# gabraham/flashpca

Measured on AMD Instinct MI355X. Metric: genotype cells/sec (N x P x iters) for k=20 PCA, higher is better.
Workload: dtype i8 (integer genotypes x 7 byte slices of the f64 operand; exact i32 accumulation, f64 recombination; agrees with the f64 kernels to ~3e-15, see fp64_mode); 1 GPU; cfg3: synthetic 500000 samples x 100000 SNPs total, SNP-sharded across GPUs, k=20 (BASELINE configs[2]/[3]); samples=500000, snps_total=100000, snps_per_gpu=100000, k=20, blockvec=16, solver_default_blockvec=16, parallelism=snp-shard x1 + all-reduce(N x b) [single]

## Files before the change

### flashpca_amd/_lib.py

```python
import ctypes as C
import os
import subprocess

HERE = os.path.dirname(os.path.abspath(__file__))
LIB_PATH = os.environ.get("FPCA_LIB") or os.path.join(HERE, "_build", "libfpca.so")
if LIB_PATH == "testhooks":
    LIB_PATH = os.path.join(HERE, "_build", "testhooks", "libfpca.so")
CLI_PATH = os.path.join(HERE, "_build", "flashpca")
HOOKS_LIB_PATH = os.path.join(HERE, "_build", "testhooks", "libfpca.so")
HOOKS_CLI_PATH = os.path.join(HERE, "_build", "testhooks", "flashpca")
CSRC = os.path.join(HERE, "csrc")

STANDARDISE = {"binom": 2, "binom2": 3}
STANDARDISE_DENSE = {"none": 0, "sd": 1, "binom": 2, "binom2": 3, "center": 4}
DIVISOR = {"none": 0, "n1": 1, "p": 2}
UNIQUE_ID_BYTES = 128
SCCA_STATUS = {0: "ok", 1: "maxiter reached", 2: "lambda1 too large", 3: "lambda2 too large"}

ALLREDUCE_FN = C.CFUNCTYPE(C.c_int, C.c_void_p, C.c_void_p, C.c_uint64, C.c_void_p)
COLLECTIVE_FN = C.CFUNCTYPE(C.c_int, C.c_void_p, C.c_void_p, C.c_void_p, C.c_uint64, C.c_void_p)


class PcaOpts(C.Structure):
    _fields_ = [
# ... 115 lines not shown
    "fpca_set_total_snps": (_I, [_P, _U64]),
    "fpca_set_rank": (_I, [_P, _I, _I]),
    "fpca_collective_stats": (_I, [_P, C.POINTER(_U64), C.POINTER(_U64)]),
    "fpca_pca_init_opts": (None, [C.POINTER(PcaOpts), C.c_size_t, C.c_size_t]),
    "fpca_pca_row_ranges": (_I, [_P, C.POINTER(PcaOpts), C.POINTER(_U64), _I]),
    "fpca_pca": (_I, [_P, C.POINTER(PcaOpts), _P, _P, _P, _P, _P, _P, C.POINTER(PcaInfo)]),
    "fpca_check": (_I, [_P, _P, C.c_int64, _P, _I, _I, _P, C.POINTER(_D), C.POINTER(_D)]),
    "fpca_ucca": (_I, [_P, _P, C.c_int64, _I, _I, _P, C.c_int64]),
    "fpca_scca_prepare": (_I, [_P, _P, C.c_int64, _I, _I, _I]),
    "fpca_scca_fit": (_I, [_P, _D, _D, _I, _I, _D, _P, C.c_int64, _P, C.c_int64, _P, C.c_int64, _P, _P, C.c_int64, _P, C.c_int64,
                           C.POINTER(_I), _P, _P, _P, C.POINTER(_I)]),
    "fpca_scca_cv": (_I, [_P, _P, C.c_int64, _I, _P, _I, _P, _I, _P, _I, _I, _I, _I, _I, _D, _P, C.c_int64, C.c_int64, _D, _I, _P, _P, _P, _P, _P, _P,
                          C.POINTER(_D), C.POINTER(_D), C.POINTER(_D), _P, _P]),
    "fpca_bench_apply": (_I, [_P, _I, _I, _I, C.POINTER(BenchResult)]),
    "fpca_profile_begin": (_I, [_P, _I]),
    "fpca_profile_sample_every": (_I, [_P, _I]),
    "fpca_profile_end": (_I, [_P, _I, C.POINTER(BenchResult), C.POINTER(_I)]),
    "fpca_bench_stats": (_I, [_P, _I, C.POINTER(_D), C.POINTER(_D)]),
    "fpca_debug_mfma_probe": (_I, [_P, _P, _P]),
    "fpca_debug_mfma_i8_probe": (_I, [_P, _P, _P]),
    "fpca_debug_mfma_peak": (_I, [_I, _I, _I, C.POINTER(_D)]),
    "fpca_debug_k4": (_I, [_P, _I, _I, _P, _P, _P, _P, _I, _P, _P]),
    "fpca_debug_k4_bench": (_I, [_P, _I, _I, _I, C.POINTER(_D), C.POINTER(_D)]),
    "fpca_debug_k4_fused": (_I, [_P, _I, _I, _P, _P, _P, _P, _P]),
    "fpca_debug_k4_fused_bench": (_I, [_P, _I, _I, _I, C.POINTER(_D)]),
    "fpca_debug_k4_inplace": (_I, [_P, _I, _I, _P, _P, _P, _I, _P, _P]),
    "fpca_debug_fp_plan": (_I, [_P, _I, C.POINTER(_I)]),
    "fpca_debug_poison_partials": (_I, [_P]),
    "fpca_debug_missing_lists": (_I, [_P, _I, _I, _P, _P, _U64, C.POINTER(_U64)]),
    "fpca_debug_gather": (_I, [_I, _I, _P, _P, _U64, _P, _U64, _P, _P, _P, _U64, _U64, _I, _D, _P, C.POINTER(_I)]),
    "fpca_debug_i8_nsc_pad": (_I, [_I, _I, C.POINTER(_I)]),
    "fpca_debug_i8_slices": (_I, [_I, _I, _I, _U64, _U64, _U64, _P, _P, _P, _P, _I, C.POINTER(SlicesOut), C.POINTER(SlicesOut), C.POINTER(_I)]),
    "fpca_debug_i8_instances": (_I, [_P, _I, C.POINTER(_I)]),
    "fpca_debug_f_sf":(_I, [_D, _U64, _I, C.POINTER(_D), C.POINTER(_D)]),
    "fpca_debug_fold_stats": (_I, [_P, _P, _I, _P, _I, _P]),
    "fpca_debug_snp_qc_rule": (_I, [_P, _P, _U64, _U64, _D, _D, _P, C.POINTER(_U64)]),
    "fpca_debug_snp_subset_bench": (_I, [_P, _P, _I, C.POINTER(_D), C.POINTER(_D)]),
    "fpca_debug_ld_prune_rule": (_I, [_P, _U64, C.c_uint32, C.c_uint32, _P, _P, _P, _P, C.POINTER(_U64)]),
    "fpca_bench_ld": (_I, [_P, C.c_uint32, _I, _P, C.POINTER(_D)]),
    "fpca_debug_king_rule": (_I, [_P, _P, _U64, _U64, _P, C.POINTER(_U64)]),
    "fpca_bench_king": (_I, [_P, _I, _P, C.POINTER(_D)]),
    "fpca_debug_sample_qc_rule": (_I, [_P, _U64, _U64, _D, _P, C.POINTER(_U64)]),
    "fpca_debug_snp_qc_counts_rule": (_I, [_P, _P, _U64, _U64, _D, _D, _D, _P, C.POINTER(_U64)]),
    "fpca_bench_qc": (_I, [_P, _I, _P, C.POINTER(_D)]),
    "fpca_debug_scratch_live": (_I, [C.POINTER(_U64)]),
    "fpca_debug_scratch_fail_at": (_I, [_U64]),
}

ABI_VERSION = 4

_lib = None
_loaded = {}


def _load(path):
    if path not in _loaded:
        if not os.path.exists(path):
            raise RuntimeError(
                "%s not found -- build it with `make -C flashpca_amd/csrc` (or __graft_entry__.build()); this package has "
                "no CPU fallback" % path
            )
        L = C.CDLL(path)
        try:
            L.fpca_abi_version.restype = C.c_int
            abi = L.fpca_abi_version()
        except AttributeError:
# ... 49 lines not shown
```

### flashpca_amd/csrc/kernels.hpp

```cpp
#pragma once
#include <hip/hip_runtime.h>

#include <cstddef>
#include <cstdint>

namespace fpca {
namespace kern {

void repitch(const uint8_t *src, uint64_t np, uint64_t nrec, uint8_t *dst, size_t pitch, hipStream_t stream);
void fix_last_byte(uint8_t *packed, size_t pitch, uint64_t np, int valid_in_last, uint64_t P_g, hipStream_t stream);
void gather_records(const uint8_t *src, size_t pitch, const uint32_t *idx, uint64_t nrec, uint8_t *dst, hipStream_t stream);
void ld_totals(const uint8_t *packed, size_t pitch, uint64_t nrec, uint32_t *tot, hipStream_t stream);
void ld_band(const uint8_t *packed, size_t pitch, const uint32_t *tot, uint32_t npad, uint64_t i0, uint64_t ni, uint64_t jend, uint32_t span,
             double *r2, uint32_t *bits, uint32_t words, double thr, bool force_general, hipStream_t stream);

void bed_stats(const uint8_t *packed, size_t pitch, uint64_t N, uint64_t P_g, int stand_method, double *lut,
               double *mean, double *sd, double *sumsq, uint32_t *nmiss , hipStream_t stream);
void lut_from_meansd(const double *mean, const double *sd, uint64_t P_g, double *lut, hipStream_t stream);

void xt_b(const uint8_t *packed, size_t pitch, const double *lut, const double *B, double *Tpart, uint64_t N_pad,
          uint64_t P_pad, int b, int nsplit, bool fp32, hipStream_t stream);
void x_t(const uint8_t *packed, size_t pitch, const double *lut, const double *T, double *Ypart, uint64_t N_pad,
         uint64_t P_pad, int b, int nsplit, bool fp32, hipStream_t stream);
void reduce_sum(const double *part, double *out, uint64_t count, int nsplit, hipStream_t stream);
// ... 39 lines not shown
void synth_generate(uint8_t *packed, size_t pitch, uint64_t N, uint64_t snp_begin, uint64_t P_g, uint64_t seed,
                    int n_pop, uint32_t fst_fp, uint32_t miss_thr, hipStream_t stream, int maf_model = 0, int missing_model = 0,
                    uint32_t conc_fp = 0, uint64_t med_q32 = 0, uint32_t sig2_fp = 0);

void mfma_layout_probe(const double *A, const double *B, double *D, hipStream_t stream);

double mfma_peak_tflops(int waves_per_simd, int iters, int pattern, hipStream_t stream);

constexpr int I8_SHARDS = 8, I8_CS_STRIDE = 640;
struct SliceOp {
   const double *rowscale;
   unsigned long long *maxbits;
   int8_t *Q;
   double *colw;
   long long *colsum;
   double *copy64;
   float *copy32;
};
void i8_colmax(const double *V, uint64_t rows, int b, int nops, const SliceOp *ops, hipStream_t stream);
void i8_slice(const double *V, uint64_t rows_pad, uint64_t rows, int b, int S, int nops, const SliceOp *ops, hipStream_t stream);
void i8_maxbits_fold(const unsigned long long *bits, double *out64, hipStream_t stream);
void i8_maxbits_set(const double *all, int G, unsigned long long *bits, hipStream_t stream);
void i8_slice_rows(const double *V, uint64_t rows, int b, int S, const SliceOp &op, int8_t *Qrm, hipStream_t stream);
void i8_unpack_slices(const int8_t *Qrm, uint64_t rows_pad, int b, int S, const SliceOp &op, hipStream_t stream, uint64_t rows_valid = 0,
                      float *copy32 = nullptr, double *copy64 = nullptr);
void i8_dequant_rows(const int8_t *Qrm, uint64_t rows, int b, int S, const SliceOp &op, float *copy32, double *copy64, hipStream_t stream);
__host__ __device__ inline size_t packed_piece_offset(uint64_t r, uint64_t q, size_t pitch, bool tiled)
{
   if (!tiled) return (size_t)(r * pitch + q * 16);
   const uint64_t c = q >> 2, kh = (q >> 1) & 1, h = q & 1;
   return (size_t)((r >> 5) * 32 * pitch + c * 2048 + (h * 64 + kh * 32 + (r & 31)) * 16);
}
int gemm_i8_nsc_pad(int S, int b);
size_t gemm_i8_workspace_doubles(uint64_t rows_pad, uint64_t k_pad, int S, int b, bool two);
int gemm_i8_instances(int (*out)[6], int cap);
void gemm_i8(const uint8_t *packed, size_t pitch, const int8_t *Qg, const int8_t *Qm, const double *wg, const double *wm,
             const long long *colsum_m, const double *mean, const double *sd, double *out, double *ws, uint64_t rows_pad, uint64_t k_pad,
             uint64_t rows_valid, int mode ,
             const double *eplane , int b, int S,
             const SliceOp *next_ops, hipStream_t stream, hipEvent_t *gemm_events = nullptr, hipEvent_t before_combine = nullptr,
             bool e_only = false ,
             bool tiled = false );
void i8_rowscales(const double *mean, const double *sd, uint64_t P_g, uint64_t P_pad, double *inv_sd, double *mu_inv_sd,
                  hipStream_t stream);
void transpose_packed(const uint8_t *in, size_t pitch_in, uint64_t N_pad, uint64_t P_pad, uint8_t *out, size_t pitch_out,
                      hipStream_t stream, bool tiled = false );
void tile_packed(const uint8_t *in, size_t pitch, uint64_t rows, uint8_t *out, hipStream_t stream);
double mfma_i8_peak_tops(int waves_per_simd, int iters, uint32_t fill, hipStream_t stream);
void mfma_i8_probe(const int8_t *A, const int8_t *Bt, int *D, hipStream_t stream);

void gather_packed_rows(const uint8_t *src, size_t pitch, const uint32_t *idx, uint32_t nidx, uint32_t rows_out, uint8_t *dst, hipStream_t stream);
void patch_missing_rows(uint8_t *packed, size_t pitch, const uint32_t *idx, uint32_t nidx, hipStream_t stream);
void scatter_packed_rows(const uint8_t *src, size_t pitch, const uint32_t *idx, uint32_t nidx, uint8_t *packed, hipStream_t stream);
void gather_scaled_rows(const double *V, const double *scale, const uint32_t *idx, uint32_t nidx, uint64_t rows_out, int b, double *dst, hipStream_t stream);
void scatter_rows(const double *src, const uint32_t *idx, uint32_t nidx, int b, double *dst, hipStream_t stream);
void count_missing(const uint8_t *packed, size_t pitch, uint64_t ncols, uint64_t nrec, uint32_t *cnt, hipStream_t stream, bool tiled = false);
void fill_missing(const uint8_t *packed, size_t pitch, uint64_t ncols, uint64_t nrec, const uint32_t *ptr, uint32_t *idx, hipStream_t stream,
                  bool tiled = false);
void sparse_rows_sum(const uint32_t *ptr, const uint32_t *idx, const double *V, const double *rowscale, int b, uint64_t nrec,
                     uint64_t rows_out, double *out, hipStream_t stream, const double *init = nullptr ,
                     bool short_lists = false ,
                     double avg_len = 0 );
void sparse_rows_sum_f32(const uint32_t *ptr, const uint32_t *idx, const float *V, const double *colw, int b, uint64_t nrec, uint64_t rows_out,
                         double *out, hipStream_t stream, const double *init = nullptr, bool short_lists = false, double avg_len = 0);
int sparse_rows_sum_variant(int b, bool rowscale, bool short_lists, double avg_len);

}
// ... 2 lines not shown
```

### flashpca_amd/csrc/kernels_i8.hip

```cpp
#include <hip/hip_runtime.h>

#include <algorithm>
#include <cmath>
#include <cstdio>
#include <cstdlib>
#include <type_traits>
#include <utility>

#include "common.hpp"
#include "dev_scratch.hpp"
#include "kernels.hpp"
#include "launch_check.hpp"

namespace fpca {
namespace kern {

typedef int v4i __attribute__((ext_vector_type(4)));
typedef int v16i __attribute__((ext_vector_type(16)));
typedef double d2 __attribute__((ext_vector_type(2)));
typedef uint32_t u4 __attribute__((ext_vector_type(4)));
typedef uint32_t u2 __attribute__((ext_vector_type(2)));



// ... 448 lines not shown
   static constexpr int SEGS = KC / 16, RSTEP = THREADS / SEGS;
   static constexpr bool HALF8 = HALF && RSTEP == 32;
   static constexpr int NP1 = HALF8 ? (COLS - 16) / RSTEP + 1 : COLS / RSTEP;
   static constexpr int NP = NQ * NP1;
   static constexpr int KS = KC / 32;
   static constexpr int PW = KC / 128;
   static constexpr int NSTEP = KS * MT * G;
   static constexpr int H = NSTEP / 2;
   static constexpr int LDS_EPI = WAVES * NT * 4096 + 2 * WC * NT * 32 * 8;
   static constexpr int LDS_NEED = (NBUF * STAGE > LDS_EPI) ? NBUF * STAGE : LDS_EPI;
   static constexpr int LDS_BYTES = (!TWO && NT <= 2 && WAVES == 4 && LDS_NEED < 56 * 1024) ? 56 * 1024 : LDS_NEED;
   static_assert((HALF8 ? (COLS - 16) % RSTEP == 0 && KC == 256 : COLS % RSTEP == 0) && NSTEP % 2 == 0 && LDS_BYTES <= 160 * 1024, "staging");
   static_assert(!HALF || RSTEP == 16 || HALF8, "the remainder tile is the last staging piece");
};

template <int MODE>
__device__ __forceinline__ bool i8_decode(uint32_t w, v4i &ag, v4i &am, uint32_t tab1)
{
   const uint32_t tabG = MODE == I8_NO_MISSING ? tab1 : 0x00010002u, tabM = 0x00000100u;
#pragma unroll
   for (int q = 0; q < 4; q++) {
      const uint32_t sel = (w >> (2 * q)) & 0x03030303u;
      ag[q] = (int)__builtin_amdgcn_perm(0u, tabG, sel);
      if (MODE != I8_NO_MISSING) am[q] = (int)__builtin_amdgcn_perm(0u, tabM, sel);
   }
   if (MODE == I8_SKIP_EMPTY)
      return __builtin_amdgcn_ballot_w64(((w & ~(w >> 1)) & 0x55555555u) != 0u) != 0ull;
   return true;
}

template <class C>
__global__ __launch_bounds__(C::THREADS, 1) void k_gemm_i8(const uint8_t *__restrict__ packed, size_t pitch,
                                                     const int8_t *__restrict__ Qg, const int8_t *__restrict__ Qm,
                                                     uint64_t k_pad, const double *__restrict__ wg, const double *__restrict__ wm, int bw,
                                                     double *__restrict__ part, uint64_t rows_pad, int chunks_total, int zb,
                                                     int nA, int sB, int cpsB, uint64_t rowB0, uint64_t rowsB, uint32_t tab1)
{
   constexpr bool TWO = C::TWO;
   constexpr int MODE = C::MODE, MATS = C::MATS;
   constexpr int MT = C::MT, NT = C::NT, NQ = C::NQ, KC = C::KC, NP = C::NP, NP1 = C::NP1, NSTEP = C::NSTEP, LDQ = C::LDQ,
                 H = C::H, G = C::G, PW = C::PW, NPK = MT * PW, NTF = C::NTF;
   constexpr bool HALF = C::HALF;
   constexpr int NBUF = C::NBUF;
   constexpr int AMASK = HALF ? 3 : 1;
   extern __shared__ __attribute__((aligned(16))) unsigned char smem[];
   const int tid = threadIdx.x, lane = tid & 63, wave = tid >> 6;
   const int li = lane & 31, kh = lane >> 5;
   const int wr = wave / C::WC, wc = wave % C::WC;
   const int rtiles = (int)((rows_pad + (C::WAVES == 8 ? C::ROWS - 1 : 0)) / C::ROWS), rtl = (rtiles + 7) / 8, ids = 8 * rtl * zb, nB = ids - nA;
   int w0 = blockIdx.x, split = 0, c_begin = 0, c_end = chunks_total;
   if (w0 >= nA) {
      const int wp = w0 - nA;
      split = wp / nB;
      w0 = nA + wp % nB;
      c_begin = split * cpsB;
      c_end = c_begin + cpsB < chunks_total ? c_begin + cpsB : chunks_total;
   }
   const int xcd = w0 & 7, sidx = w0 >> 3;
   const int zblk = sidx % zb, rt = (sidx / zb) * 8 + xcd;
   if (rt >= rtiles || c_begin >= c_end) return;
   const uint64_t row0 = (uint64_t)rt * C::ROWS;
   const int col0 = zblk * C::COLS;
   const bool idle = C::WAVES == 8 && __builtin_amdgcn_readfirstlane((int)(row0 + (uint64_t)(wr * 32 * MT) >= rows_pad)) != 0;

   v16i acc[MATS][MT][NT];
   v4i acch[MATS][MT][2];
#pragma unroll
// ... 236 lines not shown
                     acc[1][m][n] = __builtin_amdgcn_mfma_i32_32x32x32_i8(am[akey & AMASK], bq[bkey & 1][NQ - 1][j], acc[1][m][n], 0, 0, 0);
               });
            }
         }
         __builtin_amdgcn_sched_barrier(0);
         if constexpr (bkey1 != bkey) {
            wait_b(std::integral_constant<int, g1>{}, std::integral_constant<int, (bkey1 & 1)>{});
            __builtin_amdgcn_sched_barrier(0);
         }
         if constexpr (ahead) {
            wait_b(i0, i0);
            __builtin_amdgcn_sched_barrier(0);
         }
      });
      if constexpr (NBUF == 3) {
         asm volatile("s_waitcnt lgkmcnt(0)" ::: "memory");
         __builtin_amdgcn_s_barrier();
         asm volatile("" ::: "memory");
         __builtin_amdgcn_sched_barrier(0);
         buf = bufn;
      } else {
#pragma unroll
         for (int m = 0; m < MT; m++)
#pragma unroll
            for (int h = 0; h < PW; h++) {
               vm_wait<0>(pkn[m][h]);
               pk[m][h] = pkn[m][h];
            }
         __syncthreads();
      }
   }

   const int tile0 = (col0 + wc * 32 * NT) / 32;
   double *out = (split == 0 ? part + (((size_t)zblk * rows_pad + row0 + wr * 32 * MT) * 2) * bw
                             : part + (size_t)zb * rows_pad * 2 * bw +
                                  ((((size_t)(split - 1) * zb + zblk) * rowsB + (row0 - rowB0) + wr * 32 * MT) * 2) * bw) +
                 li;
   __syncthreads();
   constexpr int WREG = NT * 4096;
   double *sW = reinterpret_cast<double *>(smem + C::WAVES * WREG);
   constexpr int WCOLS = C::WC * NT * 32;
   for (int t = tid; t < WCOLS; t += C::THREADS) {
      sW[t] = t < C::COLS ? wg[col0 + t] : 0.0;
      sW[WCOLS + t] = t < C::COLS ? wm[col0 + t] : 0.0;
   }
   __syncthreads();
   static_assert(C::LDS_BYTES >= C::WAVES * WREG + 2 * WCOLS * 8, "epilogue LDS layout");
   if (idle) return;
   int *sT = reinterpret_cast<int *>(smem + wave * WREG);
   const double *sWl = sW + wc * 32 * NT + li;
   const int kb = bw / 32;
#pragma unroll
   for (int a = 0; a < MATS; a++)
#pragma unroll
      for (int m = 0; m < MT; m++) {
#pragma unroll
         for (int n = 0; n < NTF; n++) {
            const v16i v = acc[a][m][n];
#pragma unroll
            for (int r = 0; r < 16; r++) sT[(n * 32 + (r & 3) + 8 * (r >> 2) + 4 * kh) * 32 + li] = v[r];
            __builtin_amdgcn_sched_barrier(0);
         }
         if constexpr (HALF) {
#pragma unroll
            for (int t = 0; t < 2; t++)
#pragma unroll
               for (int r = 0; r < 4; r++) {
                  const int row = 16 * t + 4 * (lane >> 4) + r;
                  sT[(NTF * 32 + row) * 32 + (lane & 15)] = acch[a][m][t][r];
                  sT[(NTF * 32 + row) * 32 + 16 + (lane & 15)] = 0;
               }
         }
         __builtin_amdgcn_fence(__ATOMIC_RELEASE, "wavefront");
         __builtin_amdgcn_wave_barrier();
         for (int j = 0; j < 16; j++) {
            const int row = 16 * kh + j;
            for (int k = 0; k < kb; k++) {
               double acc64 = 0.0;
               for (int n = NT - 1 - ((NT - 1 - k) % kb); n >= 0; n -= kb)
                  acc64 += sWl[a * WCOLS + 32 * n] * (double)sT[(n * 32 + row) * 32 + li];
               out[((size_t)(32 * m + row) * 2 + a) * bw + 32 * ((tile0 + k) % kb)] = acc64;
            }
         }
         __builtin_amdgcn_fence(__ATOMIC_ACQUIRE, "wavefront");
         __builtin_amdgcn_wave_barrier();
      }
}

__global__ __launch_bounds__(256) void k_i8_combine(const double *__restrict__ part, int zb, int rows_tile, int nA, int sB, uint64_t rowB0,
                                                     uint64_t rowsB, uint64_t rows_pad, uint64_t rows_valid, int mats,
                                                     const double *__restrict__ eplane ,
                                                     int b, int bw, int S,
                                                     const double *__restrict__ wm, const long long *__restrict__ colsum_m ,
                                                     const double *__restrict__ mean, const double *__restrict__ sd,
                                                     double *__restrict__ out, const double *__restrict__ rs0,
                                                     unsigned long long *__restrict__ bits0, const double *__restrict__ rs1,
                                                     unsigned long long *__restrict__ bits1)
{
   __shared__ double smax[256], sw[9 * 64], sones[64];
   const int c = threadIdx.x % b, r_in = threadIdx.x / b, r_step = 256 / b;
   double m0 = 0.0, m1 = 0.0;
   for (int t = threadIdx.x; t < S * b; t += 256) sw[t] = (mats < 0 || !colsum_m) ? 0.0 : wm[t] * (double)colsum_fold(colsum_m, t);
   __syncthreads();
   if ((int)threadIdx.x < b) {
      double o = 0.0;
      for (int s = S - 1; s >= 0; s--) o += sw[s * b + threadIdx.x];
      sones[threadIdx.x] = o;
   }
   __syncthreads();
   if (r_in < r_step) {
      const double ones = sones[c];
      for (uint64_t row = (uint64_t)blockIdx.x * r_step + r_in; row < rows_pad; row += (uint64_t)gridDim.x * r_step) {
         double accg = 0.0, acce = 0.0;
         const int rt = (int)(row / rows_tile);
         for (int z = 0; z < zb; z++) {
            const int w0 = ((rt >> 3) * zb + z) * 8 + (rt & 7);
            const int np = w0 < nA ? 1 : sB;
            for (int p = 0; p < np; p++) {
               const double *q = p == 0 ? part + (((size_t)z * rows_pad + row) * 2) * bw
                                        : part + (size_t)zb * rows_pad * 2 * bw + ((((size_t)(p - 1) * zb + z) * rowsB + (row - rowB0)) * 2) * bw;
               for (int j = c; j < bw; j += b) {
                  accg += q[j];
                  if (mats == 2) acce += q[bw + j];
               }
            }
         }
         if (mats == 1) acce = row >= rows_valid ? ones : (eplane ? eplane[row * b + c] : 0.0);
         const double accm = ones - acce;
         double v;
         if (mats < 0)
            v = row < rows_valid ? accg : 0.0;
         else if (mean) {
            const double sdv = sd[row];
            v = (sdv > 1e-9) ? (accg - mean[row] * accm) / sdv : 0.0;
         } else
            v = accg - accm;
         out[row * b + c] = v;
         if (bits0) {
            m0 = fmax(m0, fabs(v * rs0[row]));
            m1 = fmax(m1, fabs(v * rs1[row]));
         }
      }
   }
   if (bits0) {
      colmax_commit(m0, b, smax, bits0);
      colmax_commit(m1, b, smax, bits1);
   }
}

template <class... C>
struct I8List {};
constexpr bool I8_RM = false, I8_TL = true;
constexpr bool I8_HALF = true;
template <int NT, int MODE, bool TILED, bool HALF = false>
using I8Two = I8Cfg<true, 2, NT, 4, 1, 256, 1, MODE, HALF, TILED>;
template <int NT, bool TILED, bool HALF = false, int WR = 4>
// ... 93 lines not shown
   const int tiles = (S * b + 31) / 32, cap = two ? 4 : 8;
   I8Shape sh{};
   sh.zb = (tiles + cap - 1) / cap;
   sh.nt = std::max(2, (tiles + sh.zb - 1) / sh.zb);
   sh.half = sh.zb == 1 && S * b == 32 * sh.nt - 16 && i8_rows4(two, mode, sh.nt, I8_HALF) != 0;
   sh.rows = i8_rows4(two, mode, sh.nt, sh.half);
   sh.cols = 32 * sh.nt - (sh.half ? 16 : 0);
   sh.kc = 256;
   sh.wide = i8_exists(two, mode, sh.nt, sh.half, 512, I8_RM) || i8_exists(two, mode, sh.nt, sh.half, 512, I8_TL);
   return sh;
}

constexpr bool i8_shapes_have_instances()
{
   for (int S = 2; S <= 8; S++)
      for (int b = 16; b <= 64; b += 16)
         for (int two = 0; two < 2; two++)
            for (int mode = I8_FULL; mode <= I8_NO_MISSING; mode++) {
               if (two && mode == I8_NO_MISSING) continue;
               const I8Shape sh = i8_shape_static(S, b, two, mode);
               const auto has = [&](int rows, bool tiled) {
                  return i8_find(I8Instances{}, I8Key{two != 0, mode, sh.nt, sh.half, rows, tiled},
                                 [&](auto c) { return decltype(c)::COLS == sh.cols && decltype(c)::KC == sh.kc; });
               };
               for (int tiled = 0; tiled < 2; tiled++) {
                  if (tiled && !two && mode != I8_NO_MISSING) continue;
                  if (!has(sh.rows, tiled != 0) || (sh.wide && !has(512, tiled != 0))) return false;
               }
            }
   return true;
}
static_assert(i8_shapes_have_instances(), "a shape of i8_shape_static has no k_gemm_i8 instance: see I8Instances");

static I8Shape i8_shape(int S, int b, bool two, int mode = I8_FULL, uint64_t rows_pad = 0)
{
   I8Shape sh = i8_shape_static(S, b, two, mode);
   if (rows_pad) sh.rows = i8_tile_rows(rows_pad, i8_ncu(), sh);
   return sh;
}

int gemm_i8_nsc_pad(int S, int b)
{
   const I8Shape s2 = i8_shape(S, b, false), s3 = i8_shape(S, b, true);
   return std::max(s2.zb * 32 * s2.nt, s3.zb * 32 * s3.nt);
}

struct I8Plan {
   int nA, sB, cpsB;
   uint64_t rowB0, rowsB;
   unsigned grid;
};

static bool i8_verbose()
{
   static const bool verbose = FPCA_TEST_ENV("FPCA_I8_VERBOSE") != nullptr;
   return verbose;
}

static I8Plan i8_plan(uint64_t rows_pad, uint64_t k_pad, const I8Shape &sh, int bw)
{
   static const char *env_s = FPCA_TEST_ENV("FPCA_I8_SPLITS");
   const int forced = (env_s && atoi(env_s) > 0) ? std::min(atoi(env_s), 16) : 0;
   const int ncu = i8_ncu();
   const int rtiles = (int)((rows_pad + (sh.rows == 512 ? 511 : 0)) / sh.rows), rtl = (rtiles + 7) / 8, ids = 8 * rtl * sh.zb;
   const int chunks = (int)(k_pad / sh.kc);
   const double t_chunk = 2.2e-6 * (double)sh.rows * sh.cols * sh.kc / (128.0 * 256 * 256);
   const double t_seg = 5e-6;
   const double t_row_plane = 2.0 * bw * 8 * 2 * sh.rows / 3.0e12;
   double best = 1e30;
   int best_nA = 0, best_s = 1;
   const int nA_full = ids / ncu * ncu;
   for (int pass = 0; pass < 2; pass++) {
      const int nA = pass == 0 ? 0 : (nA_full == ids ? ids - ncu : nA_full);
      if (pass == 1 && (nA <= 0 || forced)) break;
      const int nB = ids - nA;
      for (int s = 1; s <= 16 && (s == 1 || (forced ? s <= chunks : s * 4 <= chunks)); s++) {
         if (pass == 0 && forced && s != std::min(forced, std::max(chunks, 1))) continue;
         const int cps = (chunks + s - 1) / s;
         const double tA = (double)(nA / ncu) * (chunks * t_chunk + t_seg);
         const double tB = (double)((nB * s + ncu - 1) / ncu) * (cps * t_chunk + t_seg);
         const double t = tA + tB + (s > 1 ? (double)s * nB * t_row_plane : 0.0);
         if (t < best * 0.995) {
            best = t;
            best_nA = nA;
            best_s = s;
         }
      }
   }
   I8Plan p;
   p.nA = best_nA;
   p.cpsB = (chunks + best_s - 1) / best_s;
   p.sB = (chunks + p.cpsB - 1) / p.cpsB;
   const int qA = (p.nA / 8) / sh.zb;
   p.rowB0 = std::min<uint64_t>((uint64_t)qA * 8 * sh.rows, rows_pad);
   p.rowsB = rows_pad - p.rowB0;
   p.grid = (unsigned)(p.nA + (ids - p.nA) * p.sB);
   if (i8_verbose())
      std::fprintf(stderr, "[fpca] int8 GEMM plan: rows %llu K %llu tile %dx%d zb %d -> %d tile ids, %d chunks; %d unsplit + %d tiles x %d splits (%d chunks each), %u workgroups, est %.3f ms\n",
                   (unsigned long long)rows_pad, (unsigned long long)k_pad, sh.rows, sh.cols, sh.zb, ids, chunks, p.nA, ids - p.nA, p.sB, p.cpsB, p.grid,
                   best * 1e3);
   return p;
}

static int i8_bw(int b)
{
   return b == 48 ? 96 : std::max(b, 32);
}

static size_t i8_plan_doubles(const I8Plan &p, uint64_t rows_pad, int zb, int bw)
{
   return ((size_t)rows_pad + (size_t)(p.sB - 1) * p.rowsB) * zb * 2 * (size_t)bw;
}

size_t gemm_i8_workspace_doubles(uint64_t rows_pad, uint64_t k_pad, int S, int b, bool two)
{
   size_t need = 0;
   for (int mode : {(int)I8_FULL, (int)I8_SKIP_EMPTY, (int)I8_NO_MISSING}) {
      if (two && mode == I8_NO_MISSING) continue;
      const I8Shape sh = i8_shape(S, b, two, mode, rows_pad);
      const I8Plan p = i8_plan(rows_pad, k_pad, sh, i8_bw(b));
      need = std::max(need, i8_plan_doubles(p, rows_pad, sh.zb, i8_bw(b)));
   }
   return need;
}

template <class C>
static void launch_i8(const I8Plan &pl, hipStream_t stream, const uint8_t *packed, size_t pitch, const int8_t *Qg, const int8_t *Qm,
                      uint64_t k_pad, const double *wg, const double *wm, int bw, double *ws, uint64_t rows_pad, int chunks_total, int zb, uint32_t tab1)
{
   static bool attr_set = false;
   if (!attr_set) {
      (void)hipFuncSetAttribute(reinterpret_cast<const void *>(&k_gemm_i8<C>), hipFuncAttributeMaxDynamicSharedMemorySize, C::LDS_BYTES);
      attr_set = true;
   }
   hipLaunchKernelGGL(HIP_KERNEL_NAME(k_gemm_i8<C>), dim3(pl.grid), dim3(C::THREADS), C::LDS_BYTES, stream, packed, pitch, Qg, Qm, k_pad, wg, wm, bw,
                      ws, rows_pad, chunks_total, zb, pl.nA, pl.sB, pl.cpsB, pl.rowB0, pl.rowsB, tab1);
}

void gemm_i8(const uint8_t *packed, size_t pitch, const int8_t *Qg, const int8_t *Qm, const double *wg, const double *wm,
             const long long *colsum_m, const double *mean, const double *sd, double *out, double *ws, uint64_t rows_pad, uint64_t k_pad,
             uint64_t rows_valid, int mode, const double *eplane , int b,
             int S, const SliceOp *next_ops ,
             hipStream_t stream, hipEvent_t *gemm_events ,
             hipEvent_t before_combine ,
             bool e_only ,
             bool tiled )
{
   const bool two = (Qg != Qm);
   if (tiled && !two && mode != I8_NO_MISSING) throw Error(-1, "gemm_i8: the one-operand kernels of both matrices read the row-major layout only");
   if (tiled && (pitch % 64 || k_pad > 4 * pitch)) throw Error(-1, "gemm_i8: a band-tiled copy has whole 64-byte chunks per row");
   if (e_only && (mode != I8_NO_MISSING || two)) throw Error(-1, "gemm_i8: e_only goes with the one-matrix kernel");
   const I8Shape sh = i8_shape(S, b, two, mode, rows_pad);
   const int bw = i8_bw(b);
   const I8Plan pl = i8_plan(rows_pad, k_pad, sh, bw);
   const int chunks_total = (int)(k_pad / sh.kc);
   if (i8_verbose())
      std::fprintf(stderr, "[fpca] int8 GEMM launch: %s, mode %d, nt %d%s, %s%s; phase B from row %llu\n", two ? "two operands" : "one operand", mode,
                   sh.nt, sh.half ? " (half tile)" : "", tiled ? "band-tiled" : "row-major", e_only ? ", E alone" : "", (unsigned long long)pl.rowB0);
   static const bool poison = FPCA_TEST_ENV("FPCA_DEBUG_I8_POISON") != nullptr;
   if (poison) {
      const size_t used = i8_plan_doubles(pl, rows_pad, sh.zb, bw);
      if (hipMemsetAsync(ws, 0xFF, used * sizeof(double), stream) != hipSuccess) throw Error(-3, "gemm_i8: poisoning the workspace failed");
   }
   if (gemm_events) (void)hipEventRecord(gemm_events[0], stream);
   if (two && mode == I8_NO_MISSING) throw Error(-1, "gemm_i8: without missing genotypes both matrices share one operand (pass Qm == Qg)");
   const bool launched = i8_find(I8Instances{}, I8Key{two, mode, sh.nt, sh.half, sh.rows, tiled}, [&](auto c) {
      using C = decltype(c);
      if (C::COLS != sh.cols || C::KC != sh.kc) throw Error(-1, "gemm_i8: the kernel instance and the shape disagree about the tile");
      launch_i8<C>(pl, stream, packed, pitch, Qg, Qm, k_pad, wg, wm, bw, ws, rows_pad, chunks_total, sh.zb, (e_only ? 0x00000100u : 0x00010002u));
      return true;
   });
   if (!launched) throw Error(-1, "gemm_i8: no kernel instance for this shape");
   launch_check();
   if (gemm_events) (void)hipEventRecord(gemm_events[1], stream);
   if (before_combine) (void)hipStreamWaitEvent(stream, before_combine, 0);
   const unsigned blocks = (unsigned)std::min<uint64_t>(1024, (rows_pad + (256 / b) - 1) / (256 / b));
   hipLaunchKernelGGL(k_i8_combine, dim3(blocks), dim3(256), 0, stream, ws, sh.zb, sh.rows, pl.nA, pl.sB, pl.rowB0, pl.rowsB, rows_pad, rows_valid, e_only ? -1 : mode == I8_NO_MISSING ? 1 : 2, eplane, b, bw, S, wm, colsum_m,
                      mean, sd, out,
                      next_ops ? next_ops[0].rowscale : nullptr, next_ops ? next_ops[0].maxbits : nullptr,
                      next_ops ? next_ops[1].rowscale : nullptr, next_ops ? next_ops[1].maxbits : nullptr);
   launch_check();
}

__global__ void k_i8_rowscales(const double *__restrict__ mean, const double *__restrict__ sd, uint64_t P_g, uint64_t P_pad,
                               double *__restrict__ inv_sd, double *__restrict__ mu_inv_sd)
{
   const uint64_t j = (uint64_t)blockIdx.x * 256 + threadIdx.x;
   if (j >= P_pad) return;
   double a = 0.0, m = 0.0;
   if (j < P_g && sd[j] > 1e-9) {
      a = 1.0 / sd[j];
      m = mean[j] / sd[j];
   }
   inv_sd[j] = a;
   mu_inv_sd[j] = m;
}

void i8_rowscales(const double *mean, const double *sd, uint64_t P_g, uint64_t P_pad, double *inv_sd, double *mu_inv_sd,
                  hipStream_t stream)
{
   hipLaunchKernelGGL(k_i8_rowscales, dim3((unsigned)((P_pad + 255) / 256)), dim3(256), 0, stream, mean, sd, P_g, P_pad, inv_sd, mu_inv_sd);
   launch_check();
}

template <bool TILED>
__global__ __launch_bounds__(256) void k_transpose_packed(const uint8_t *__restrict__ in, size_t pitch_in, uint8_t *__restrict__ out,
                                                           size_t pitch_out)
{
   __shared__ uint32_t tile[256][17];
   const uint64_t snp0 = (uint64_t)blockIdx.x * 256, smp0 = (uint64_t)blockIdx.y * 256;
// ... 264 lines not shown
```

### include/fpca_debug.h

```cpp
#ifndef FPCA_DEBUG_H
#define FPCA_DEBUG_H

#include "fpca.h"

#ifdef __cplusplus
extern "C" {
#endif

typedef struct fpca_bench_result {
   double ms_total;
   double ms_xt;
   double ms_x;
   double ms_allreduce;
   double flops_per_step;
   double packed_bytes_per_step;
   double ms_gemm_xt;
   double ms_gemm_x;
} fpca_bench_result;
int fpca_bench_apply(fpca_ctx *ctx, int b, int steps, int warmup, fpca_bench_result *res);
int fpca_profile_begin(fpca_ctx *ctx, int max_steps);
int fpca_profile_sample_every(fpca_ctx *ctx, int stride);
int fpca_profile_end(fpca_ctx *ctx, int b, fpca_bench_result *res, int *nsteps);
int fpca_bench_stats(fpca_ctx *ctx, int reps, double *ms_per_launch, double *bytes_per_launch);

// ... 4 lines not shown
                  double *Out, double *G_out);
int fpca_debug_k4_fused(fpca_ctx *ctx, int b, int nq, const double *V, const double *W, const double *C_in, double *Out, double *Cg);
int fpca_debug_k4_fused_bench(fpca_ctx *ctx, int b, int nq, int reps, double *ms_fused);
int fpca_debug_k4_inplace(fpca_ctx *ctx, int b, int nq, const double *V, const double *W, const double *C_in, int mode, double *Out,
                          double *G_out);
int fpca_debug_k4_bench(fpca_ctx *ctx, int b, int nq, int reps, double *ms_gram, double *ms_gemm);

int fpca_debug_fp_plan(fpca_ctx *ctx, int b, int out[6]);
int fpca_debug_poison_partials(fpca_ctx *ctx);

int fpca_debug_missing_lists(fpca_ctx *ctx, int b, int by_sample, uint32_t *ptr_out, uint32_t *idx_out, uint64_t idx_cap, uint64_t *nnz);
int fpca_debug_gather(int b, int use_f32, const uint32_t *ptr, const uint32_t *idx, uint64_t nnz, const void *V, uint64_t v_rows,
                      const double *rowscale, const double *colw, const double *init, uint64_t nrec, uint64_t rows_out, int short_lists,
                      double avg_len, double *out, int *variant);

typedef struct fpca_debug_slices_out {
   double *colmax;
   uint64_t *maxbits_own;
   uint64_t *maxbits;
   int8_t *Q;
   int8_t *Qrm;
   double *colw;
   int64_t *colsum;
   float *copy32;
   double *copy64;
   float *dq32;
   double *dq64;
} fpca_debug_slices_out;
int fpca_debug_i8_nsc_pad(int S, int b, int *nsc_pad);
int fpca_debug_i8_slices(int route, int b, int S, uint64_t rows, uint64_t rows_pad, uint64_t rows_valid, const double *V, const double *rowscale0,
                         const double *rowscale1, const double *peers, int n_peers, fpca_debug_slices_out *out0, fpca_debug_slices_out *out1,
                         int *nsc_pad);
int fpca_debug_i8_instances(int32_t *keys, int cap, int *count);

int fpca_debug_f_sf(double r2, uint64_t n, int k, double *F, double *P);
int fpca_debug_fold_stats(fpca_ctx *ctx, const uint8_t *fold, int nfolds, uint32_t *counts, int which_fold, double *mean_sd);
int fpca_debug_snp_qc_rule(const double *mean, const uint32_t *n_missing, uint64_t N, uint64_t P, double min_maf, double max_missing,
                           uint8_t *keep, uint64_t *n_kept);
int fpca_debug_snp_subset_bench(fpca_ctx *src, const uint8_t *keep, int reps, double *ms_per_launch, double *bytes_per_launch);
int fpca_debug_ld_prune_rule(const uint32_t *bits, uint64_t P, uint32_t window, uint32_t step, const uint64_t *totals, const double *maf,
                             const uint32_t *chrom, uint8_t *keep, uint64_t *n_kept);
int fpca_bench_ld(fpca_ctx *ctx, uint32_t span, int reps, double *ms, double *macs);
int fpca_debug_king_rule(const uint32_t *i, const uint32_t *j, uint64_t n_pairs, uint64_t N, uint8_t *keep, uint64_t *n_kept);
int fpca_bench_king(fpca_ctx *ctx, int reps, double *ms, double *macs);
int fpca_debug_sample_qc_rule(const uint32_t *counts, uint64_t n_snps, uint64_t N, double max_missing, uint8_t *samples, uint64_t *n_kept);
int fpca_debug_snp_qc_counts_rule(const uint32_t *counts, const double *p_hwe, uint64_t n, uint64_t P, double min_maf, double max_missing,
                                  double min_hwe_p, uint8_t *keep, uint64_t *n_kept);
int fpca_bench_qc(fpca_ctx *ctx, int reps, double *ms, double *hwe_steps);

int fpca_debug_scratch_live(uint64_t out[3]);
int fpca_debug_scratch_fail_at(uint64_t n);

#ifdef __cplusplus
}
#endif
#endif
```

Before: 79830 billion cells/s.

## Fold b=16 int8 GEMM partials across half-waves and size workspace per matrix count

For block width 16 the int8 GEMM epilogue now sums the two 16-lane halves of each 32-column tile with a permlane16 swap and stores only 16 doubles per row. It also drops the unused second plane for the one-matrix (no-missing) mode, which shrinks partial-sum writes and combine reads. The split planner's per-row plane cost is updated to match, and a new rule skips the phase-B split when the tail would fill too many CUs. The change adds cross-lane shuffles, a debug plan-query entry point and an env override, and relies on every layout index being changed consistently between kernel and combine.

```diff
diff --git a/flashpca_amd/_lib.py b/flashpca_amd/_lib.py
--- a/flashpca_amd/_lib.py
+++ b/flashpca_amd/_lib.py
@@ -171,6 +171,7 @@
     "fpca_debug_i8_nsc_pad": (_I, [_I, _I, C.POINTER(_I)]),
     "fpca_debug_i8_slices": (_I, [_I, _I, _I, _U64, _U64, _U64, _P, _P, _P, _P, _I, C.POINTER(SlicesOut), C.POINTER(SlicesOut), C.POINTER(_I)]),
     "fpca_debug_i8_instances": (_I, [_P, _I, C.POINTER(_I)]),
+    "fpca_debug_i8_plan": (_I, [_U64, _U64, _I, _I, _I, _I, _I, _P, C.POINTER(_U64)]),
     "fpca_debug_f_sf":(_I, [_D, _U64, _I, C.POINTER(_D), C.POINTER(_D)]),
     "fpca_debug_fold_stats": (_I, [_P, _P, _I, _P, _I, _P]),
     "fpca_debug_snp_qc_rule": (_I, [_P, _P, _U64, _U64, _D, _D, _P, C.POINTER(_U64)]),
diff --git a/flashpca_amd/csrc/kernels.hpp b/flashpca_amd/csrc/kernels.hpp
--- a/flashpca_amd/csrc/kernels.hpp
+++ b/flashpca_amd/csrc/kernels.hpp
@@ -95,7 +95,8 @@
    return (size_t)((r >> 5) * 32 * pitch + c * 2048 + (h * 64 + kh * 32 + (r & 31)) * 16);
 }
 int gemm_i8_nsc_pad(int S, int b);
-size_t gemm_i8_workspace_doubles(uint64_t rows_pad, uint64_t k_pad, int S, int b, bool two);
+size_t gemm_i8_workspace_doubles(uint64_t rows_pad, uint64_t k_pad, int S, int b, bool two, int ncu = 0 );
+void gemm_i8_plan_numbers(uint64_t rows_pad, uint64_t k_pad, int S, int b, bool two, int mode, int ncu, long long out[13]);
 int gemm_i8_instances(int (*out)[6], int cap);
 void gemm_i8(const uint8_t *packed, size_t pitch, const int8_t *Qg, const int8_t *Qm, const double *wg, const double *wm,
              const long long *colsum_m, const double *mean, const double *sd, double *out, double *ws, uint64_t rows_pad, uint64_t k_pad,
diff --git a/flashpca_amd/csrc/kernels_i8.hip b/flashpca_amd/csrc/kernels_i8.hip
--- a/flashpca_amd/csrc/kernels_i8.hip
+++ b/flashpca_amd/csrc/kernels_i8.hip
@@ -504,7 +504,7 @@
 template <class C>
 __global__ __launch_bounds__(C::THREADS, 1) void k_gemm_i8(const uint8_t *__restrict__ packed, size_t pitch,
                                                      const int8_t *__restrict__ Qg, const int8_t *__restrict__ Qm,
-                                                     uint64_t k_pad, const double *__restrict__ wg, const double *__restrict__ wm, int bw,
+                                                     uint64_t k_pad, const double *__restrict__ wg, const double *__restrict__ wm, int bwc,
                                                      double *__restrict__ part, uint64_t rows_pad, int chunks_total, int zb,
                                                      int nA, int sB, int cpsB, uint64_t rowB0, uint64_t rowsB, uint32_t tab1)
 {
@@ -807,9 +807,11 @@
    }
 
    const int tile0 = (col0 + wc * 32 * NT) / 32;
-   double *out = (split == 0 ? part + (((size_t)zblk * rows_pad + row0 + wr * 32 * MT) * 2) * bw
-                             : part + (size_t)zb * rows_pad * 2 * bw +
-                                  ((((size_t)(split - 1) * zb + zblk) * rowsB + (row0 - rowB0) + wr * 32 * MT) * 2) * bw) +
+   const bool fold = bwc < 32;
+   const int rstride = MATS * bwc;
+   double *out = (split == 0 ? part + ((size_t)zblk * rows_pad + row0 + wr * 32 * MT) * rstride
+                             : part + (size_t)zb * rows_pad * rstride +
+                                  (((size_t)(split - 1) * zb + zblk) * rowsB + (row0 - rowB0) + wr * 32 * MT) * rstride) +
                  li;
    __syncthreads();
    constexpr int WREG = NT * 4096;
@@ -824,7 +826,7 @@
    if (idle) return;
    int *sT = reinterpret_cast<int *>(smem + wave * WREG);
    const double *sWl = sW + wc * 32 * NT + li;
-   const int kb = bw / 32;
+   const int kb = fold ? 1 : bwc / 32;
 #pragma unroll
    for (int a = 0; a < MATS; a++)
 #pragma unroll
@@ -854,7 +856,13 @@
                double acc64 = 0.0;
                for (int n = NT - 1 - ((NT - 1 - k) % kb); n >= 0; n -= kb)
                   acc64 += sWl[a * WCOLS + 32 * n] * (double)sT[(n * 32 + row) * 32 + li];
-               out[((size_t)(32 * m + row) * 2 + a) * bw + 32 * ((tile0 + k) % kb)] = acc64;
+               if (fold) {
+                  const unsigned long long u = (unsigned long long)__double_as_longlong(acc64);
+                  const auto pl = __builtin_amdgcn_permlane16_swap((unsigned)u, (unsigned)u, false, false);
+                  const auto ph = __builtin_amdgcn_permlane16_swap((unsigned)(u >> 32), (unsigned)(u >> 32), false, false);
+                  acc64 += __longlong_as_double((long long)(((unsigned long long)ph[1] << 32) | pl[1]));
+               }
+               if (!fold || li < 16) out[((size_t)(32 * m + row) * MATS + a) * bwc + 32 * ((tile0 + k) % kb)] = acc64;
             }
          }
          __builtin_amdgcn_fence(__ATOMIC_ACQUIRE, "wavefront");
@@ -865,7 +873,7 @@
 __global__ __launch_bounds__(256) void k_i8_combine(const double *__restrict__ part, int zb, int rows_tile, int nA, int sB, uint64_t rowB0,
                                                      uint64_t rowsB, uint64_t rows_pad, uint64_t rows_valid, int mats,
                                                      const double *__restrict__ eplane ,
-                                                     int b, int bw, int S,
+                                                     int b, int bwc, int S,
                                                      const double *__restrict__ wm, const long long *__restrict__ colsum_m ,
                                                      const double *__restrict__ mean, const double *__restrict__ sd,
                                                      double *__restrict__ out, const double *__restrict__ rs0,
@@ -874,6 +882,7 @@
 {
    __shared__ double smax[256], sw[9 * 64], sones[64];
    const int c = threadIdx.x % b, r_in = threadIdx.x / b, r_step = 256 / b;
+   const int rstride = (mats == 2 ? 2 : 1) * bwc;
    double m0 = 0.0, m1 = 0.0;
    for (int t = threadIdx.x; t < S * b; t += 256) sw[t] = (mats < 0 || !colsum_m) ? 0.0 : wm[t] * (double)colsum_fold(colsum_m, t);
    __syncthreads();
@@ -892,11 +901,11 @@
             const int w0 = ((rt >> 3) * zb + z) * 8 + (rt & 7);
             const int np = w0 < nA ? 1 : sB;
             for (int p = 0; p < np; p++) {
-               const double *q = p == 0 ? part + (((size_t)z * rows_pad + row) * 2) * bw
-                                        : part + (size_t)zb * rows_pad * 2 * bw + ((((size_t)(p - 1) * zb + z) * rowsB + (row - rowB0)) * 2) * bw;
-               for (int j = c; j < bw; j += b) {
+               const double *q = p == 0 ? part + ((size_t)z * rows_pad + row) * rstride
+                                        : part + (size_t)zb * rows_pad * rstride + (((size_t)(p - 1) * zb + z) * rowsB + (row - rowB0)) * rstride;
+               for (int j = c; j < bwc; j += b) {
                   accg += q[j];
-                  if (mats == 2) acce += q[bw + j];
+                  if (mats == 2) acce += q[bwc + j];
                }
             }
          }
@@ -1056,10 +1065,10 @@
 }
 static_assert(i8_shapes_have_instances(), "a shape of i8_shape_static has no k_gemm_i8 instance: see I8Instances");
 
-static I8Shape i8_shape(int S, int b, bool two, int mode = I8_FULL, uint64_t rows_pad = 0)
+static I8Shape i8_shape(int S, int b, bool two, int mode = I8_FULL, uint64_t rows_pad = 0, int ncu = 0 )
 {
    I8Shape sh = i8_shape_static(S, b, two, mode);
-   if (rows_pad) sh.rows = i8_tile_rows(rows_pad, i8_ncu(), sh);
+   if (rows_pad) sh.rows = i8_tile_rows(rows_pad, ncu ? ncu : i8_ncu(), sh);
    return sh;
 }
 
@@ -1075,22 +1084,41 @@
    unsigned grid;
 };
 
+constexpr double I8_PLANE_RATE = 2.7e12;
+constexpr double I8_TAIL_FILL_MAX = 0.75;
+
 static bool i8_verbose()
 {
    static const bool verbose = FPCA_TEST_ENV("FPCA_I8_VERBOSE") != nullptr;
    return verbose;
 }
 
-static I8Plan i8_plan(uint64_t rows_pad, uint64_t k_pad, const I8Shape &sh, int bw)
+static int i8_bw(int b)
+{
+   return b == 48 ? 96 : std::max(b, 32);
+}
+
+static int i8_bwc(int b)
+{
+   return b == 16 ? 16 : i8_bw(b);
+}
+static int i8_row_doubles(int b, int mode)
+{
+   return (mode == I8_NO_MISSING ? 1 : 2) * i8_bwc(b);
+}
+
+static I8Plan i8_plan(uint64_t rows_pad, uint64_t k_pad, const I8Shape &sh, int row_doubles, int ncu_arg = 0 )
 {
    static const char *env_s = FPCA_TEST_ENV("FPCA_I8_SPLITS");
    const int forced = (env_s && atoi(env_s) > 0) ? std::min(atoi(env_s), 16) : 0;
-   const int ncu = i8_ncu();
+   static const char *env_b = FPCA_TEST_ENV("FPCA_I8_PHASEB");
+   const int forcedB = (!forced && env_b && atoi(env_b) > 0) ? std::min(atoi(env_b), 16) : 0;
+   const int ncu = ncu_arg ? ncu_arg : i8_ncu();
    const int rtiles = (int)((rows_pad + (sh.rows == 512 ? 511 : 0)) / sh.rows), rtl = (rtiles + 7) / 8, ids = 8 * rtl * sh.zb;
    const int chunks = (int)(k_pad / sh.kc);
    const double t_chunk = 2.2e-6 * (double)sh.rows * sh.cols * sh.kc / (128.0 * 256 * 256);
    const double t_seg = 5e-6;
-   const double t_row_plane = 2.0 * bw * 8 * 2 * sh.rows / 3.0e12;
+   const double t_row_plane = 2.0 * row_doubles * 8 * sh.rows / I8_PLANE_RATE;
    double best = 1e30;
    int best_nA = 0, best_s = 1;
    const int nA_full = ids / ncu * ncu;
@@ -1098,6 +1126,7 @@
       const int nA = pass == 0 ? 0 : (nA_full == ids ? ids - ncu : nA_full);
       if (pass == 1 && (nA <= 0 || forced)) break;
       const int nB = ids - nA;
+      if (pass == 1 && nB > I8_TAIL_FILL_MAX * ncu) break;
       for (int s = 1; s <= 16 && (s == 1 || (forced ? s <= chunks : s * 4 <= chunks)); s++) {
          if (pass == 0 && forced && s != std::min(forced, std::max(chunks, 1))) continue;
          const int cps = (chunks + s - 1) / s;
@@ -1109,6 +1138,13 @@
             best_nA = nA;
             best_s = s;
          }
+      }
+   }
+   if (forcedB) {
+      const int nA = nA_full == ids ? ids - ncu : nA_full;
+      if (nA > 0) {
+         best_nA = nA;
+         best_s = std::max(1, std::min(forcedB, chunks));
       }
    }
    I8Plan p;
@@ -1126,38 +1162,44 @@
    return p;
 }
 
-static int i8_bw(int b)
-{
-   return b == 48 ? 96 : std::max(b, 32);
-}
-
-static size_t i8_plan_doubles(const I8Plan &p, uint64_t rows_pad, int zb, int bw)
-{
-   return ((size_t)rows_pad + (size_t)(p.sB - 1) * p.rowsB) * zb * 2 * (size_t)bw;
-}
-
-size_t gemm_i8_workspace_doubles(uint64_t rows_pad, uint64_t k_pad, int S, int b, bool two)
+static size_t i8_plan_doubles(const I8Plan &p, uint64_t rows_pad, int zb, int row_doubles)
+{
+   return ((size_t)rows_pad + (size_t)(p.sB - 1) * p.rowsB) * zb * (size_t)row_doubles;
+}
+
+size_t gemm_i8_workspace_doubles(uint64_t rows_pad, uint64_t k_pad, int S, int b, bool two, int ncu)
 {
    size_t need = 0;
    for (int mode : {(int)I8_FULL, (int)I8_SKIP_EMPTY, (int)I8_NO_MISSING}) {
       if (two && mode == I8_NO_MISSING) continue;
-      const I8Shape sh = i8_shape(S, b, two, mode, rows_pad);
-      const I8Plan p = i8_plan(rows_pad, k_pad, sh, i8_bw(b));
-      need = std::max(need, i8_plan_doubles(p, rows_pad, sh.zb, i8_bw(b)));
+      const I8Shape sh = i8_shape(S, b, two, mode, rows_pad, ncu);
+      const I8Plan p = i8_plan(rows_pad, k_pad, sh, i8_row_doubles(b, mode), ncu);
+      need = std::max(need, i8_plan_doubles(p, rows_pad, sh.zb, i8_row_doubles(b, mode)));
    }
    return need;
+}
+
+void gemm_i8_plan_numbers(uint64_t rows_pad, uint64_t k_pad, int S, int b, bool two, int mode, int ncu, long long out[13])
+{
+   const I8Shape sh = i8_shape(S, b, two, mode, rows_pad, ncu);
+   const I8Plan p = i8_plan(rows_pad, k_pad, sh, i8_row_doubles(b, mode), ncu);
+   const int rtiles = (int)((rows_pad + (sh.rows == 512 ? 511 : 0)) / sh.rows);
+   const long long v[13] = {sh.rows, sh.cols, sh.zb, 8 * ((rtiles + 7) / 8) * sh.zb, (long long)(k_pad / sh.kc), p.nA, p.sB, p.cpsB, (long long)p.rowB0,
+                            (long long)p.rowsB, (long long)p.grid, (long long)i8_plan_doubles(p, rows_pad, sh.zb, i8_row_doubles(b, mode)),
+                            i8_row_doubles(b, mode)};
+   std::copy(v, v + 13, out);
 }
 
 template <class C>
 static void launch_i8(const I8Plan &pl, hipStream_t stream, const uint8_t *packed, size_t pitch, const int8_t *Qg, const int8_t *Qm,
-                      uint64_t k_pad, const double *wg, const double *wm, int bw, double *ws, uint64_t rows_pad, int chunks_total, int zb, uint32_t tab1)
+                      uint64_t k_pad, const double *wg, const double *wm, int bwc, double *ws, uint64_t rows_pad, int chunks_total, int zb, uint32_t tab1)
 {
    static bool attr_set = false;
    if (!attr_set) {
       (void)hipFuncSetAttribute(reinterpret_cast<const void *>(&k_gemm_i8<C>), hipFuncAttributeMaxDynamicSharedMemorySize, C::LDS_BYTES);
       attr_set = true;
    }
-   hipLaunchKernelGGL(HIP_KERNEL_NAME(k_gemm_i8<C>), dim3(pl.grid), dim3(C::THREADS), C::LDS_BYTES, stream, packed, pitch, Qg, Qm, k_pad, wg, wm, bw,
+   hipLaunchKernelGGL(HIP_KERNEL_NAME(k_gemm_i8<C>), dim3(pl.grid), dim3(C::THREADS), C::LDS_BYTES, stream, packed, pitch, Qg, Qm, k_pad, wg, wm, bwc,
                       ws, rows_pad, chunks_total, zb, pl.nA, pl.sB, pl.cpsB, pl.rowB0, pl.rowsB, tab1);
 }
 
@@ -1175,15 +1217,15 @@
    if (tiled && (pitch % 64 || k_pad > 4 * pitch)) throw Error(-1, "gemm_i8: a band-tiled copy has whole 64-byte chunks per row");
    if (e_only && (mode != I8_NO_MISSING || two)) throw Error(-1, "gemm_i8: e_only goes with the one-matrix kernel");
    const I8Shape sh = i8_shape(S, b, two, mode, rows_pad);
-   const int bw = i8_bw(b);
-   const I8Plan pl = i8_plan(rows_pad, k_pad, sh, bw);
+   const int bwc = i8_bwc(b), row_doubles = i8_row_doubles(b, mode);
+   const I8Plan pl = i8_plan(rows_pad, k_pad, sh, row_doubles);
    const int chunks_total = (int)(k_pad / sh.kc);
    if (i8_verbose())
       std::fprintf(stderr, "[fpca] int8 GEMM launch: %s, mode %d, nt %d%s, %s%s; phase B from row %llu\n", two ? "two operands" : "one operand", mode,
                    sh.nt, sh.half ? " (half tile)" : "", tiled ? "band-tiled" : "row-major", e_only ? ", E alone" : "", (unsigned long long)pl.rowB0);
    static const bool poison = FPCA_TEST_ENV("FPCA_DEBUG_I8_POISON") != nullptr;
    if (poison) {
-      const size_t used = i8_plan_doubles(pl, rows_pad, sh.zb, bw);
+      const size_t used = i8_plan_doubles(pl, rows_pad, sh.zb, row_doubles);
       if (hipMemsetAsync(ws, 0xFF, used * sizeof(double), stream) != hipSuccess) throw Error(-3, "gemm_i8: poisoning the workspace failed");
    }
    if (gemm_events) (void)hipEventRecord(gemm_events[0], stream);
@@ -1191,7 +1233,8 @@
    const bool launched = i8_find(I8Instances{}, I8Key{two, mode, sh.nt, sh.half, sh.rows, tiled}, [&](auto c) {
       using C = decltype(c);
       if (C::COLS != sh.cols || C::KC != sh.kc) throw Error(-1, "gemm_i8: the kernel instance and the shape disagree about the tile");
-      launch_i8<C>(pl, stream, packed, pitch, Qg, Qm, k_pad, wg, wm, bw, ws, rows_pad, chunks_total, sh.zb, (e_only ? 0x00000100u : 0x00010002u));
+      static_assert(C::MATS == (C::MODE == I8_NO_MISSING ? 1 : 2), "i8_row_doubles counts the matrices the instance writes");
+      launch_i8<C>(pl, stream, packed, pitch, Qg, Qm, k_pad, wg, wm, bwc, ws, rows_pad, chunks_total, sh.zb, (e_only ? 0x00000100u : 0x00010002u));
       return true;
    });
    if (!launched) throw Error(-1, "gemm_i8: no kernel instance for this shape");
@@ -1199,7 +1242,7 @@
    if (gemm_events) (void)hipEventRecord(gemm_events[1], stream);
    if (before_combine) (void)hipStreamWaitEvent(stream, before_combine, 0);
    const unsigned blocks = (unsigned)std::min<uint64_t>(1024, (rows_pad + (256 / b) - 1) / (256 / b));
-   hipLaunchKernelGGL(k_i8_combine, dim3(blocks), dim3(256), 0, stream, ws, sh.zb, sh.rows, pl.nA, pl.sB, pl.rowB0, pl.rowsB, rows_pad, rows_valid, e_only ? -1 : mode == I8_NO_MISSING ? 1 : 2, eplane, b, bw, S, wm, colsum_m,
+   hipLaunchKernelGGL(k_i8_combine, dim3(blocks), dim3(256), 0, stream, ws, sh.zb, sh.rows, pl.nA, pl.sB, pl.rowB0, pl.rowsB, rows_pad, rows_valid, e_only ? -1 : mode == I8_NO_MISSING ? 1 : 2, eplane, b, bwc, S, wm, colsum_m,
                       mean, sd, out,
                       next_ops ? next_ops[0].rowscale : nullptr, next_ops ? next_ops[0].maxbits : nullptr,
                       next_ops ? next_ops[1].rowscale : nullptr, next_ops ? next_ops[1].maxbits : nullptr);
diff --git a/include/fpca_debug.h b/include/fpca_debug.h
--- a/include/fpca_debug.h
+++ b/include/fpca_debug.h
@@ -60,6 +60,7 @@
                          const double *rowscale1, const double *peers, int n_peers, fpca_debug_slices_out *out0, fpca_debug_slices_out *out1,
                          int *nsc_pad);
 int fpca_debug_i8_instances(int32_t *keys, int cap, int *count);
+int fpca_debug_i8_plan(uint64_t rows_pad, uint64_t k_pad, int S, int b, int two, int mode, int ncu, int64_t *plan, uint64_t *workspace_doubles);
 
 int fpca_debug_f_sf(double r2, uint64_t n, int k, double *F, double *P);
 int fpca_debug_fold_stats(fpca_ctx *ctx, const uint8_t *fold, int nfolds, uint32_t *counts, int which_fold, double *mean_sd);
```

Measured after the change: 79880 billion cells/s, median of 2. About the same (+0.1%).
